# ai4co/rl4co

Measured on AMD Instinct MI355X. Metric: decode_steps_per_sec, higher is better.
Workload: dtype bf16; 1 GPU; BASELINE configs[1]: TSPEnv num_loc=100 batch=4096/GPU AttentionModel(3L,d128,h8) greedy rollout, bf16 encoder GEMMs, bf16 cache; leg=c2_greedy, batch_per_gpu=4096, cache_dtype=bf16, launch=pipeline, input=one synthetic batch resident in HBM, reused by every step, parallelism=replicas x1 (instances sharded)

## Files before the change

rl4co_amd/csrc/am_decode.hip:

```cpp
#include <hip/hip_runtime.h>

#include "common.h"
#include "rl4co_math.h"
#include "topkp.h"

namespace {

constexpr int kD = RL4CO_EMBED_DIM;
constexpr int kH = RL4CO_NUM_HEADS;
constexpr int kDH = kD / kH;
constexpr int kUnroll = 4;
constexpr float kNegInf = -__builtin_huge_valf();
constexpr float kSqrtD = 11.3137084989847604f;

struct CacheF32 {
  using elem = float;
  using raw = float4;
  static constexpr int EPL = 4;
  __device__ static inline raw zero() { return make_float4(0.f, 0.f, 0.f, 0.f); }
  __device__ static inline raw ld(const elem* p) { return *reinterpret_cast<const float4*>(p); }
  __device__ static inline void cvt(const raw& t, float (&v)[4]) {
    v[0] = t.x; v[1] = t.y; v[2] = t.z; v[3] = t.w;
  }
};
// ... 8 lines not shown
    v[0] = __uint_as_float(t.x << 16); v[1] = __uint_as_float(t.x & 0xffff0000u);
    v[2] = __uint_as_float(t.y << 16); v[3] = __uint_as_float(t.y & 0xffff0000u);
    v[4] = __uint_as_float(t.z << 16); v[5] = __uint_as_float(t.z & 0xffff0000u);
    v[6] = __uint_as_float(t.w << 16); v[7] = __uint_as_float(t.w & 0xffff0000u);
  }
};

struct CacheF16 {
  using elem = uint16_t;
  using raw = uint4;
  static constexpr int EPL = 8;
  typedef _Float16 half2_t __attribute__((ext_vector_type(2)));
  __device__ static inline raw zero() { return make_uint4(0u, 0u, 0u, 0u); }
  __device__ static inline raw ld(const elem* p) { return *reinterpret_cast<const uint4*>(p); }
  __device__ static inline void cvt(const raw& t, float (&v)[8]) {
    const half2_t a = __builtin_bit_cast(half2_t, t.x), b = __builtin_bit_cast(half2_t, t.y);
    const half2_t c = __builtin_bit_cast(half2_t, t.z), d = __builtin_bit_cast(half2_t, t.w);
    v[0] = (float)a[0]; v[1] = (float)a[1]; v[2] = (float)b[0]; v[3] = (float)b[1];
    v[4] = (float)c[0]; v[5] = (float)c[1]; v[6] = (float)d[0]; v[7] = (float)d[1];
  }
};

__host__ __device__ inline int lds_pad(int N) { return (N + 63) & ~63; }

template <class C>
struct CtxTables {
  const char *cur, *first;
  int64_t rs;
  bool half;
  __device__ inline CtxTables(const rl4co_am_decode_args& a, int cb, int N, int e0) {
    half = a.ctx_dtype != RL4CO_DT_F32;
    const int64_t esz = half ? 2 : 4;
    rs = (a.ctx_row_stride ? a.ctx_row_stride : (int64_t)kD) * esz;
    const int64_t off = ((int64_t)cb * (a.ctx_batch_stride ? a.ctx_batch_stride : (int64_t)N * kD) + e0) * esz;
    cur = a.ctx_cur ? static_cast<const char*>(a.ctx_cur) + off : nullptr;
    first = a.ctx_first ? static_cast<const char*>(a.ctx_first) + off : nullptr;
  }
  __device__ inline void load(const char* table, int64_t row, float (&v)[C::EPL]) const {
    const char* p = table + row * rs;
    if constexpr (sizeof(typename C::elem) == 2) {
      if (half) {
        C::cvt(C::ld(reinterpret_cast<const typename C::elem*>(p)), v);
        return;
      }
    }
#pragma unroll
    for (int e = 0; e < C::EPL; ++e) v[e] = reinterpret_cast<const float*>(p)[e];
  }
};

__device__ inline int trajectory_of_block(int b, int B, int B_inst) {
  const int S = B / B_inst;
  if (S == 1 || (B_inst & 7) != 0) return b;
  const int xcd = b & 7, k = b >> 3;
  return (k % S) * B_inst + (k / S) * 8 + xcd;
}

__device__ inline void wave_lds_sync() {
  __builtin_amdgcn_fence(__ATOMIC_RELEASE, "workgroup");
  __builtin_amdgcn_wave_barrier();
  __builtin_amdgcn_fence(__ATOMIC_ACQUIRE, "workgroup");
}

struct TrajState {
  int cur, first;
  long long step_i;
  float used;
  float time;
  bool done;
  uint32_t errbits;
  float ent_acc;
};

__device__ inline int build_list(const rl4co_am_decode_args& a, const uint8_t* mk, uint16_t* fl, int N, int lane) {
  int F = 0;
  if (a.mask_inner && a.mask_logits) {
    for (int j0 = 0; j0 < N; j0 += 64) {
      const int j = j0 + lane;
      const bool f = j < N && mk[j] != 0;
      const unsigned long long bal = __ballot(f);
      if (f) fl[F + __popcll(bal & ((1ull << lane) - 1ull))] = (uint16_t)j;
      F += __popcll(bal);
    }
  } else {
    for (int j = lane; j < N; j += 64) fl[j] = (uint16_t)j;
    F = N;
  }
  wave_lds_sync();
  return F;
}

template <int ENV>
__device__ inline int commit_and_step(const rl4co_am_decode_args& a, TrajState& st, float* lg, const uint16_t* fl, int F,
                                      uint8_t* mk, uint8_t* vis, const float* dem, float cap, int r, int t, int N, int lane,
                                      const float* oplocs, const float* opmax, const float* twdur, int bc);

template <int ENV, bool FILT = false>
__device__ inline int finalize_and_step(const rl4co_am_decode_args& a, TrajState& st, float* lg, float* xs,
                                        const uint16_t* fl, int F, uint8_t* mk, uint8_t* vis, const float* dem, float cap,
                                        int r, int t, int N, int lane, const float* oplocs = nullptr,
                                        const float* opmax = nullptr, const float* twdur = nullptr) {
  bool nan_seen = false;
  float zmax = kNegInf;
  for (int c = lane; c < F; c += 64) {
    float z = lg[c] / kSqrtD;
    if (z != z) nan_seen = true;
    if (a.tanh_clipping > 0.0f) z = rl4co_tanhf(z) * a.tanh_clipping;
    if (a.mask_logits && mk[fl[c]] == 0) z = kNegInf;
    if (a.temperature != 1.0f) z = z / a.temperature;
    lg[c] = z;
    zmax = fmaxf(zmax, z);
  }
  if (__any(nan_seen)) st.errbits |= RL4CO_EBIT_NAN_LOGIT;
  zmax = rl4co::bfly_max<1, 64>(zmax);
  float zsum = 0.0f;
  const int64_t tcol = (int64_t)a.t0 + t;
  constexpr bool filt = FILT;
  if (filt) {
    for (int c = lane; c < F; c += 64) xs[c] = rl4co_expf(lg[c] - zmax);
    zsum = rl4co::topkp_filter(lg, xs, F, a.top_k, a.top_p, lane);
    if (a.kept_bits)
      rl4co::topkp_write_bits(a.kept_bits + ((int64_t)r * a.out_stride + tcol) * a.kept_words, a.kept_words, lg, fl, F,
                              N, reinterpret_cast<uint32_t*>(xs + N), lane);
  } else {
    for (int c = lane; c < F; c += 64) zsum = zsum + rl4co_expf(lg[c] - zmax);
    zsum = rl4co::bfly_sum<1, 64>(zsum);
  }
  const float lse = rl4co_logf(zsum);

  float best = kNegInf;
  int bc = 0x7fffffff;
  float ent = 0.0f;
  float* alp = a.all_logps ? a.all_logps + ((int64_t)r * a.out_stride + tcol) * N : nullptr;
  if (alp && F < N) {
    for (int j = lane; j < N; j += 64)
      if (mk[j] == 0) alp[j] = kNegInf;
  }
  for (int c = lane; c < F; c += 64) {
    const int j = fl[c];
    const float lp = (lg[c] - zmax) - lse;
    lg[c] = lp;
    float key = lp;
    if (a.mode == RL4CO_DECODE_SAMPLE) {
      const float nz = a.exp_noise
                           ? a.exp_noise[((int64_t)t * a.B + r) * N + j]
                           : rl4co_exp1_noise(a.philox_seed ^ (a.philox_seed_dev ? *a.philox_seed_dev : 0ull),
                                              a.philox_offset + (uint64_t)tcol, (uint32_t)r,
                                              (uint32_t)j);
      key = rl4co_expf(lp) / nz;
      if (filt && !(lp > kNegInf)) key = kNegInf;
    }
    if (bc == 0x7fffffff || key > best) {
      best = key;
      bc = c;
    }
    if (a.entropy && lp > kNegInf) ent = fmaf(rl4co_expf(lp), lp, ent);
    if (alp) alp[j] = lp;
  }
  rl4co::bfly_argmax(best, bc);
  if (a.entropy) st.ent_acc = st.ent_acc - rl4co::bfly_sum<1, 64>(ent);
  wave_lds_sync();
  return commit_and_step<ENV>(a, st, lg, fl, F, mk, vis, dem, cap, r, t, N, lane, oplocs, opmax, twdur, bc);
}

template <int ENV>
__device__ inline int commit_and_step(const rl4co_am_decode_args& a, TrajState& st, float* lg, const uint16_t* fl, int F,
                                      uint8_t* mk, uint8_t* vis, const float* dem, float cap, int r, int t, int N, int lane,
                                      const float* oplocs, const float* opmax, const float* twdur, int bc) {
  const int64_t tcol = (int64_t)a.t0 + t;
  int bi;
  float logp;
  if (a.mode == RL4CO_DECODE_EVALUATE) {
    bi = (int)a.forced_actions[(int64_t)r * a.out_stride + tcol];
    if (bi < 0 || bi >= N) {
      st.errbits |= RL4CO_EBIT_INFEASIBLE;
      bi = 0;
    }
    int pos = 0x7fffffff;
    for (int c = lane; c < F; c += 64)
      if (fl[c] == bi) pos = c;
    pos = -rl4co::bfly_i_max(-pos);
    logp = pos < F ? lg[pos] : kNegInf;
  } else {
    bi = (bc < F) ? (int)fl[bc] : 0;
    logp = (bc < F) ? lg[bc] : kNegInf;
  }
  if (mk[bi] == 0) st.errbits |= RL4CO_EBIT_INFEASIBLE;
  if (!(logp > -1000.0f)) st.errbits |= RL4CO_EBIT_NEG_INF_LOGP;
  if (lane == 0) {
    a.actions[(int64_t)r * a.out_stride + tcol] = bi;
    a.logps[(int64_t)r * a.out_stride + tcol] = logp;
  }
  wave_lds_sync();

  if (ENV == RL4CO_ENV_TSP) {
    if (st.step_i == 0) st.first = bi;
    st.cur = bi;
    if (lane == 0) mk[bi] = 0;
    st.step_i += 1;
    wave_lds_sync();
    bool any_left = false;
    for (int j = lane; j < N; j += 64) any_left |= mk[j] != 0;
    st.done = !__any(any_left);
  } else if (ENV == RL4CO_ENV_PDP) {
    const int n = N - 1;
    if (lane == 0) {
      vis[bi] &= (uint8_t)~1u;
      vis[(bi + n / 2) % (n + 1)] |= 2;
    }
    st.step_i += 1;
    st.cur = bi;
    wave_lds_sync();
    bool left = false;
    for (int j = lane; j < N; j += 64) {
      const uint8_t v = vis[j];
      mk[j] = (v == 3) ? 1 : 0;
      left |= (v & 1) != 0;
    }
    st.done = !__any(left);
  } else if (ENV == RL4CO_ENV_PCTSP) {
    st.used = st.used + dem[bi];
    if (lane == 0) vis[bi] = 1;
    st.done = (bi == 0) && (st.step_i > 0);
    st.step_i += 1;
    st.cur = bi;
    wave_lds_sync();
    const bool depot_visited = vis[0] != 0;
    bool unvisited = false;
    for (int j = lane; j < N; j += 64) {
      if (j >= 1) {
        mk[j] = (vis[j] != 0 || depot_visited) ? 0 : 1;
        unvisited |= vis[j] == 0;
      }
    }
    unvisited = __any(unvisited);
    if (lane == 0) mk[0] = ((st.used < 1.0f) && unvisited) ? 0 : 1;
  } else if (ENV == RL4CO_ENV_OP) {
    const float cx = oplocs[2 * st.cur], cy = oplocs[2 * st.cur + 1];
    const float bx = oplocs[2 * bi], by = oplocs[2 * bi + 1];
    {
      const float dx = bx - cx, dy = by - cy;
      st.used = st.used + sqrtf(fmaf(dy, dy, dx * dx));
    }
    if (lane == 0) vis[bi] = 1;
    st.done = (bi == 0) && (st.step_i > 0);
    st.step_i += 1;
    st.cur = bi;
    wave_lds_sync();
    const bool depot_visited = vis[0] != 0;
    for (int j = lane; j < N; j += 64) {
      const float dx = oplocs[2 * j] - bx, dy = oplocs[2 * j + 1] - by;
      const bool exceeds = st.used + sqrtf(fmaf(dy, dy, dx * dx)) > opmax[j];
      mk[j] = (j == 0 || !(vis[j] != 0 || depot_visited || exceeds)) ? 1 : 0;
    }
  } else {
    if (ENV == RL4CO_ENV_CVRPTW) {
      const float dx = oplocs[2 * bi] - oplocs[2 * st.cur], dy = oplocs[2 * bi + 1] - oplocs[2 * st.cur + 1];
      const float served = fmaxf(st.time + sqrtf(fmaf(dy, dy, dx * dx)), opmax[2 * bi]) + twdur[bi];
      st.time = (bi != 0 ? 1.0f : 0.0f) * served;
    }
    const int di = min(max(bi - 1, 0), N - 2);
    st.used = (st.used + dem[di]) * (bi != 0 ? 1.0f : 0.0f);
    st.cur = bi;
    if (lane == 0) vis[bi] = 1;
    wave_lds_sync();
    const float thr = cap + 1e-5f;
    bool any_feasible = false, all_visited = true;
    for (int j = lane; j < N; j += 64) {
      all_visited &= vis[j] != 0;
      if (j >= 1) {
        const bool masked = (vis[j] != 0) || (dem[j - 1] + st.used > thr);
        mk[j] = masked ? 0 : 1;
        any_feasible |= !masked;
      }
    }
    any_feasible = __any(any_feasible);
    st.done = __all(all_visited);
    if (lane == 0) mk[0] = ((st.cur == 0) && any_feasible) ? 0 : 1;
    if (ENV == RL4CO_ENV_CVRPTW) {
      wave_lds_sync();
      const float bx = oplocs[2 * bi], by = oplocs[2 * bi + 1];
      for (int j = lane; j < N; j += 64) {
        const float dx = oplocs[2 * j] - bx, dy = oplocs[2 * j + 1] - by;
        if (!(st.time + sqrtf(fmaf(dy, dy, dx * dx)) <= opmax[2 * j + 1])) mk[j] = 0;
      }
    }
  }
  wave_lds_sync();
  return bi;
}

template <int EPL>
__device__ inline void gemv_t(float (&out)[EPL], const float* __restrict__ wt, const float* in_lds, int width, int e0) {
#pragma unroll
  for (int e = 0; e < EPL; ++e) out[e] = 0.0f;
  for (int k = 0; k < width; ++k) {
    const float c = in_lds[k];
#pragma unroll
    for (int e = 0; e < EPL; ++e) out[e] = fmaf(wt[(int64_t)k * kD + e0 + e], c, out[e]);
  }
}

constexpr int kRowCacheNone = 0xFF;
__host__ __device__ inline int row_cache_bytes(int N, int S, int esz) {
  return S > 0 ? S * 3 * kD * esz + lds_pad(N) + S : 0;
}

template <class C, int ENV, bool UNFOLD = false, bool FILT = false>
__global__ void __launch_bounds__(64) am_decode_kernel(const rl4co_am_decode_args a, const int S) {
  constexpr int EPL = C::EPL;
  constexpr int LPR = kD / EPL;
  constexpr int RPL = 64 / LPR;
  constexpr int LPH = kDH / EPL;
  constexpr bool kRowCache = !UNFOLD && (ENV == RL4CO_ENV_TSP || ENV == RL4CO_ENV_CVRP);
  using elem = typename C::elem;
  using raw_t = typename C::raw;

  extern __shared__ __align__(16) unsigned char smem[];
  const int lane = threadIdx.x;
  const int r = trajectory_of_block(blockIdx.x, a.B, a.B_inst);
  const int N = a.N;
  const int Np = lds_pad(N);
  float* sc = reinterpret_cast<float*>(smem);
  float* lg = sc + Np * kH;
  float* mh = lg + Np;
  uint16_t* fl = reinterpret_cast<uint16_t*>(mh + kH);
  uint8_t* mk = reinterpret_cast<uint8_t*>(fl + Np);
  uint8_t* vis = mk + Np;
  elem* rc = reinterpret_cast<elem*>(vis + Np);
  uint8_t* rslot = reinterpret_cast<uint8_t*>(rc + S * 3 * kD);
  uint8_t* rpend = rslot + Np;

  const int cb = r % a.B_inst;
  const int rg = lane / LPR;
  const int li = lane % LPR;
  const int hd = li / LPH;
  const int e0 = li * EPL;

  const elem* Kg = static_cast<const elem*>(a.glimpse_key) + (int64_t)cb * a.kvl_batch_stride + e0;
  const elem* Vg = static_cast<const elem*>(a.glimpse_val) + (int64_t)cb * a.kvl_batch_stride + e0;
  const elem* Kl = static_cast<const elem*>(a.logit_key) + (int64_t)cb * a.kvl_batch_stride + e0;
  const int64_t rs = a.kvl_row_stride;
  const CtxTables<C> ctx(a, cb, N, e0);
  const float* hrow = UNFOLD ? a.node_embed + (int64_t)cb * N * kD + e0 : nullptr;

  uint8_t* gmask = a.action_mask + (int64_t)r * N;
  for (int j = lane; j < Np; j += 64) mk[j] = (j < N) ? gmask[j] : (uint8_t)0;
  constexpr bool kScalarCtx = ENV == RL4CO_ENV_CVRP || ENV == RL4CO_ENV_OP || ENV == RL4CO_ENV_PCTSP || ENV == RL4CO_ENV_CVRPTW;
  constexpr bool kCvrpLike = ENV == RL4CO_ENV_CVRP || ENV == RL4CO_ENV_CVRPTW;
  if (ENV == RL4CO_ENV_PDP) {
    const uint8_t* gv = a.visited + (int64_t)r * N;
    const uint8_t* gt = a.to_deliver + (int64_t)r * N;
    for (int j = lane; j < Np; j += 64) vis[j] = (j < N) ? (uint8_t)((gv[j] != 0 ? 1 : 0) | (gt[j] != 0 ? 2 : 0)) : (uint8_t)0;
  } else if (ENV != RL4CO_ENV_TSP) {
    const uint8_t* gv = a.visited + (int64_t)r * N;
    for (int j = lane; j < Np; j += 64) vis[j] = (j < N) ? gv[j] : (uint8_t)1;
  }
  TrajState st;
  st.cur = (int)a.current_node[r];
  st.first = (ENV == RL4CO_ENV_TSP) ? (int)a.first_node[r] : 0;
  st.step_i = !kCvrpLike ? a.step_i[r] : 0;
  st.time = (ENV == RL4CO_ENV_CVRPTW) ? a.current_time[r] : 0.0f;
  st.used = kScalarCtx ? a.used_capacity[r] : 0.0f;
  st.done = a.done[r] != 0;
  st.errbits = 0;
  st.ent_acc = 0.0f;
  const float* oplocs = (ENV == RL4CO_ENV_OP || ENV == RL4CO_ENV_CVRPTW) ? a.locs + (int64_t)cb * N * 2 : nullptr;
  const float* opmax = (ENV == RL4CO_ENV_OP)       ? a.max_length + (int64_t)cb * N
                       : (ENV == RL4CO_ENV_CVRPTW) ? a.time_windows + (int64_t)cb * N * 2
                                                   : nullptr;
  const float* twdur = (ENV == RL4CO_ENV_CVRPTW) ? a.durations + (int64_t)cb * N : nullptr;
  const float cap = (kCvrpLike || ENV == RL4CO_ENV_PCTSP) ? a.vehicle_capacity[r]
                                                                      : ((ENV == RL4CO_ENV_OP) ? opmax[0] : 0.0f);
  const float* dem = kCvrpLike                  ? a.demand + (int64_t)cb * (N - 1)
                     : (ENV == RL4CO_ENV_PCTSP) ? a.demand + (int64_t)cb * N
                                                : nullptr;
  wave_lds_sync();

  const bool list_all = !(a.mask_inner && a.mask_logits);
  auto candidate = [&](int j) -> bool {
    return list_all || (ENV == RL4CO_ENV_TSP ? mk[j] != 0 : (j == 0 || vis[j] == 0));
  };
  const bool caching = kRowCache && S > 0;
  if (caching) {
    for (int j = lane; j < Np; j += 64) rslot[j] = (uint8_t)kRowCacheNone;
    wave_lds_sync();
    int k = 0;
    for (int j0 = N - 1; j0 >= 0 && k < S; j0 -= 64) {
      const int j = j0 - lane;
      const bool f = j >= 0 && candidate(j);
      const unsigned long long bal = __ballot(f);
      const int s = k + __popcll(bal & ((1ull << lane) - 1ull));
      if (f && s < S) {
        rslot[j] = (uint8_t)s;
        rpend[s] = 1;
      }
      k += __popcll(bal);
    }
    wave_lds_sync();
  }
  auto lds_row = [&](int j, int plane) -> const elem* { return rc + (rslot[j] * 3 + plane) * kD + e0; };
  auto fill_row = [&](int j, int plane, const raw_t& v) {
    const int s = rslot[j];
    if (s != kRowCacheNone) *reinterpret_cast<raw_t*>(rc + (s * 3 + plane) * kD + e0) = v;
  };

  float qb[EPL];
#pragma unroll
  for (int e = 0; e < EPL; ++e) qb[e] = a.q_bias ? a.q_bias[(int64_t)cb * kD + e0 + e] : 0.0f;

  const bool single = a.max_steps == 1;
  int t = 0;
  int rows_read = 0;

  for (; t < a.max_steps && (!st.done || single); ++t) {
    const int F = build_list(a, mk, fl, N, lane);
    int hend = F, pbeg = F;
    if (caching) {
      const int c_lo = max(F - S, 0);
      int last_hbm = c_lo - 1, first_pend = F;
      for (int c = c_lo + lane; c < F; c += 64) {
        const int s = rslot[fl[c]];
        const bool pend = s != kRowCacheNone && rpend[s] != 0;
        if (s == kRowCacheNone || pend) last_hbm = c;
        if (pend) first_pend = min(first_pend, c);
      }
      hend = rl4co::bfly_i_max(last_hbm) + 1;
      pbeg = -rl4co::bfly_i_max(-first_pend);
    }
    rows_read += hend;

    float q[EPL];
    if constexpr (UNFOLD) {
      float* cv = sc;
      if (rg == 0) {
        if (ENV == RL4CO_ENV_TSP) {
          const bool ph = st.step_i < 1;
#pragma unroll
          for (int e = 0; e < EPL; ++e) {
            cv[e0 + e] = ph ? a.w_placeholder[e0 + e] : hrow[(int64_t)st.first * kD + e];
            cv[kD + e0 + e] = ph ? a.w_placeholder[kD + e0 + e] : hrow[(int64_t)st.cur * kD + e];
          }
        } else {
#pragma unroll
          for (int e = 0; e < EPL; ++e) cv[e0 + e] = hrow[(int64_t)st.cur * kD + e];
          if (li == 0) cv[kD] = cap - st.used;
        }
      }
      wave_lds_sync();
      gemv_t<EPL>(q, a.w_ctx_t, cv, a.ctx_width, e0);
#pragma unroll
      for (int e = 0; e < EPL; ++e) q[e] = q[e] + qb[e];
      wave_lds_sync();
    } else if (ENV == RL4CO_ENV_TSP) {
      if (st.step_i < 1) {
#pragma unroll
        for (int e = 0; e < EPL; ++e) q[e] = a.q_step0[e0 + e] + qb[e];
      } else {
        float cf[EPL], cc[EPL];
        ctx.load(ctx.first, st.first, cf);
        ctx.load(ctx.cur, st.cur, cc);
#pragma unroll
        for (int e = 0; e < EPL; ++e) q[e] = (cf[e] + cc[e]) + qb[e];
      }
    } else if (ENV == RL4CO_ENV_PDP) {
      float cc[EPL];
      ctx.load(ctx.cur, st.cur, cc);
#pragma unroll
      for (int e = 0; e < EPL; ++e) q[e] = cc[e] + qb[e];
    } else {
      float rem = cap - st.used;
      if (ENV == RL4CO_ENV_PCTSP && !(rem > 0.0f)) rem = 0.0f;
      float cc[EPL];
      ctx.load(ctx.cur, st.cur, cc);
#pragma unroll
      for (int e = 0; e < EPL; ++e) {
        float v = fmaf(a.w_cap[e0 + e], rem, cc[e]);
        if (ENV == RL4CO_ENV_CVRPTW) v = fmaf(a.w_time[e0 + e], st.time, v);
        q[e] = v + qb[e];
      }
    }
#pragma unroll
    for (int e = 0; e < EPL; ++e) q[e] = q[e] * 0.25f;

    float m = kNegInf;
    auto score = [&](const raw_t& rw, int c, int j) {
      const bool valid = j >= 0;
      float k[EPL];
      C::cvt(rw, k);
      float acc = 0.0f;
#pragma unroll
      for (int e = 0; e < EPL; ++e) acc = fmaf(q[e], k[e], acc);
      acc = rl4co::bfly_sum<1, LPH>(acc);
      const bool feas = valid && (!a.mask_inner || mk[valid ? j : 0] != 0);
      const float sv = feas ? acc : kNegInf;
      if (valid && (li % LPH) == 0) sc[c * kH + hd] = sv;
      m = fmaxf(m, sv);
    };
    for (int c0 = 0; c0 < F; c0 += RPL * kUnroll) {
      raw_t rw[kUnroll];
      int jj[kUnroll];
#pragma unroll
      for (int u = 0; u < kUnroll; ++u) {
        const int c = c0 + u * RPL + rg;
        jj[u] = (c < F) ? (int)fl[c] : -1;
        rw[u] = (jj[u] < 0) ? C::zero() : (c < hend ? C::ld(Kg + (int64_t)jj[u] * rs) : C::ld(lds_row(jj[u], 0)));
      }
#pragma unroll
      for (int u = 0; u < kUnroll; ++u) {
        const int c = c0 + u * RPL + rg;
        if (caching && c >= pbeg && c < hend) fill_row(jj[u], 0, rw[u]);
        score(rw[u], c, jj[u]);
      }
    }
    m = rl4co::bfly_max<LPR, 64>(m);
    if (rg == 0 && (li % LPH) == 0) mh[hd] = m;
    wave_lds_sync();
    {
      const float mm = mh[lane & (kH - 1)];
      for (int idx = lane; idx < F * kH; idx += 64) sc[idx] = rl4co_expf(sc[idx] - mm);
    }
    wave_lds_sync();

    float l = 0.0f;
    float o[EPL];
#pragma unroll
    for (int e = 0; e < EPL; ++e) o[e] = 0.0f;
    auto accumulate = [&](const raw_t& rw, int c, bool ok) {
      float v[EPL];
      C::cvt(rw, v);
      const float p = ok ? sc[c * kH + hd] : 0.0f;
      l = l + p;
#pragma unroll
      for (int e = 0; e < EPL; ++e) o[e] = fmaf(p, v[e], o[e]);
    };
    for (int c0 = 0; c0 < F; c0 += RPL * kUnroll) {
      raw_t rw[kUnroll];
      bool ok[kUnroll];
#pragma unroll
      for (int u = 0; u < kUnroll; ++u) {
        const int c = c0 + u * RPL + rg;
        ok[u] = c < F;
        rw[u] = !ok[u] ? C::zero() : (c < hend ? C::ld(Vg + (int64_t)fl[c] * rs) : C::ld(lds_row(fl[c], 1)));
      }
#pragma unroll
      for (int u = 0; u < kUnroll; ++u) {
        const int c = c0 + u * RPL + rg;
        if (caching && c >= pbeg && c < hend) fill_row(fl[c], 1, rw[u]);
        accumulate(rw[u], c, ok[u]);
      }
    }
    l = 1.0f / rl4co::bfly_sum<LPR, 64>(l);
#pragma unroll
    for (int e = 0; e < EPL; ++e) o[e] = rl4co::bfly_sum<LPR, 64>(o[e]) * l;
    if constexpr (UNFOLD) {
      wave_lds_sync();
      if (rg == 0) {
#pragma unroll
        for (int e = 0; e < EPL; ++e) sc[e0 + e] = o[e];
      }
      wave_lds_sync();
      gemv_t<EPL>(o, a.w_out_t, sc, kD, e0);
    }

    auto logit = [&](const raw_t& rw, int c) {
      float k[EPL];
      C::cvt(rw, k);
      float acc = 0.0f;
#pragma unroll
      for (int e = 0; e < EPL; ++e) acc = fmaf(o[e], k[e], acc);
      acc = rl4co::bfly_sum<1, LPR>(acc);
      if (c < F && li == 0) lg[c] = acc;
    };
    for (int c0 = 0; c0 < F; c0 += RPL * kUnroll) {
      raw_t rw[kUnroll];
#pragma unroll
      for (int u = 0; u < kUnroll; ++u) {
        const int c = c0 + u * RPL + rg;
        rw[u] = (c >= F) ? C::zero() : (c < hend ? C::ld(Kl + (int64_t)fl[c] * rs) : C::ld(lds_row(fl[c], 2)));
      }
#pragma unroll
      for (int u = 0; u < kUnroll; ++u) {
        const int c = c0 + u * RPL + rg;
        if (caching && c >= pbeg && c < hend) fill_row(fl[c], 2, rw[u]);
        logit(rw[u], c);
      }
    }
    if (caching) {
      for (int c = pbeg + lane; c < hend; c += 64) {
        const int s = rslot[fl[c]];
        if (s != kRowCacheNone) rpend[s] = 0;
      }
    }
    wave_lds_sync();

    const int bi = finalize_and_step<ENV, FILT>(a, st, lg, sc, fl, F, mk, vis, dem, cap, r, t, N, lane, oplocs, opmax, twdur);
    if (caching && rslot[bi] != kRowCacheNone && !candidate(bi)) {
      int nxt = -1;
      for (int j = lane; j < N; j += 64)
        if (candidate(j) && rslot[j] == kRowCacheNone) nxt = j;
      nxt = rl4co::bfly_i_max(nxt);
      const int s = rslot[bi];
      wave_lds_sync();
      if (lane == 0) {
        rslot[bi] = (uint8_t)kRowCacheNone;
        if (nxt >= 0) {
          rslot[nxt] = (uint8_t)s;
          rpend[s] = 1;
        }
      }
      wave_lds_sync();
    }
  }
  if (!single && !st.done && t >= a.max_steps) st.errbits |= RL4CO_EBIT_MAX_STEPS;

  for (int j = lane; j < N; j += 64) gmask[j] = mk[j];
  if (ENV == RL4CO_ENV_PDP) {
    uint8_t* gv = a.visited + (int64_t)r * N;
    uint8_t* gt = a.to_deliver + (int64_t)r * N;
    for (int j = lane; j < N; j += 64) {
      gv[j] = vis[j] & 1;
      gt[j] = (vis[j] >> 1) & 1;
    }
  } else if (ENV != RL4CO_ENV_TSP) {
    uint8_t* gv = a.visited + (int64_t)r * N;
    for (int j = lane; j < N; j += 64) gv[j] = vis[j];
  }
  if (lane == 0) {
    a.current_node[r] = st.cur;
    a.done[r] = st.done ? 1 : 0;
    if (ENV == RL4CO_ENV_TSP) a.first_node[r] = st.first;
    if (!kCvrpLike) a.step_i[r] = st.step_i;
    if (ENV == RL4CO_ENV_CVRPTW) a.current_time[r] = st.time;
    if (kScalarCtx) a.used_capacity[r] = st.used;
    if (a.n_steps) a.n_steps[r] = t;
    if (a.steps_summary) {
      atomicMax(a.steps_summary, t);
      atomicAdd(a.steps_summary + 1, t);
      atomicAdd(reinterpret_cast<unsigned long long*>(a.steps_summary + 2), (unsigned long long)rows_read);
    }
    if (a.entropy) a.entropy[r] += st.ent_acc;
    if (st.errbits) atomicOr(a.err, (int)st.errbits);
  }
}

constexpr int kLdsWaves = 4;
constexpr int kLdsGroups = 16;

template <int ENV, bool FILT = false>
__device__ inline int wide_scores(const rl4co_am_decode_args& a, TrajState& st, float* lg, const uint16_t* fl, int F,
                                  const uint8_t* mk, float* xs, int nw, int r, int t, int N, int tid) {
  constexpr int T = 64 * kLdsWaves;
  const int w = tid >> 6, lane = tid & 63;
  float* ex = xs;
  float* xw = xs + 2 * nw;
  bool nan_seen = false;
  float zmax = kNegInf;
  for (int c = tid; c < F; c += T) {
    float z = lg[c] / kSqrtD;
    if (z != z) nan_seen = true;
    if (a.tanh_clipping > 0.0f) z = rl4co_tanhf(z) * a.tanh_clipping;
    if (a.mask_logits && mk[fl[c]] == 0) z = kNegInf;
    if (a.temperature != 1.0f) z = z / a.temperature;
    lg[c] = z;
    zmax = fmaxf(zmax, z);
  }
  zmax = rl4co::bfly_max<1, 64>(zmax);
  const bool wave_nan = __any(nan_seen);
  if (lane == 0) {
    xw[w] = zmax;
    xw[4 + w] = wave_nan ? 1.0f : 0.0f;
  }
  __syncthreads();
  zmax = fmaxf(fmaxf(xw[0], xw[1]), fmaxf(xw[2], xw[3]));
  if ((xw[4] + xw[5]) + (xw[6] + xw[7]) != 0.0f) st.errbits |= RL4CO_EBIT_NAN_LOGIT;
  for (int c = tid; c < F; c += T) ex[c] = rl4co_expf(lg[c] - zmax);
  __syncthreads();
  const int64_t tcol = (int64_t)a.t0 + t;
  constexpr bool filt = FILT;
  if (w == 0) {
    float zsum = 0.0f;
    if (filt) {
      zsum = rl4co::topkp_filter(lg, ex, F, a.top_k, a.top_p, lane);
      if (a.kept_bits)
        rl4co::topkp_write_bits(a.kept_bits + ((int64_t)r * a.out_stride + tcol) * a.kept_words, a.kept_words, lg, fl,
                                F, N, reinterpret_cast<uint32_t*>(xw + 16), lane);
    } else {
      for (int c = lane; c < F; c += 64) zsum = zsum + ex[c];
      zsum = rl4co::bfly_sum<1, 64>(zsum);
    }
    if (lane == 0) xw[8] = rl4co_logf(zsum);
  }
  __syncthreads();
  const float lse = xw[8];
  float* alp = a.all_logps ? a.all_logps + ((int64_t)r * a.out_stride + tcol) * N : nullptr;
  if (alp && F < N) {
    for (int j = tid; j < N; j += T)
      if (mk[j] == 0) alp[j] = kNegInf;
  }
  for (int c = tid; c < F; c += T) {
    const int j = fl[c];
    const float lp = (lg[c] - zmax) - lse;
    lg[c] = lp;
    float key = lp;
    if (a.mode == RL4CO_DECODE_SAMPLE) {
      const float nz = a.exp_noise
                           ? a.exp_noise[((int64_t)t * a.B + r) * N + j]
                           : rl4co_exp1_noise(a.philox_seed ^ (a.philox_seed_dev ? *a.philox_seed_dev : 0ull),
                                              a.philox_offset + (uint64_t)tcol, (uint32_t)r,
                                              (uint32_t)j);
      key = rl4co_expf(lp) / nz;
      if (filt && !(lp > kNegInf)) key = kNegInf;
    }
    ex[c] = key;
    if (alp) alp[j] = lp;
  }
  __syncthreads();
  int bc = 0x7fffffff;
  if (w == 0) {
    float best = kNegInf, ent = 0.0f;
    for (int c = lane; c < F; c += 64) {
      const float key = ex[c];
      if (bc == 0x7fffffff || key > best) {
        best = key;
        bc = c;
      }
      if (a.entropy) {
        const float lp = lg[c];
        if (lp > kNegInf) ent = fmaf(rl4co_expf(lp), lp, ent);
      }
    }
    rl4co::bfly_argmax(best, bc);
    if (a.entropy) st.ent_acc = st.ent_acc - rl4co::bfly_sum<1, 64>(ent);
    wave_lds_sync();
  }
  return bc;
}

__host__ __device__ inline int lds_variant_sc_rows(int N) { return N < 80 ? 80 : N; }
__host__ __device__ inline int wide_scratch_bytes(int N) {
  const int nw = (N + 3) & ~3;
  return lds_variant_sc_rows(N) * kH * 4 + nw * 4 + kLdsWaves * kH * 4 + 32 + 2 * nw + 2 * nw;
}
__host__ __device__ inline int lds_variant_bytes(int N) { return 3 * N * kD * 2 + wide_scratch_bytes(N); }

template <int ENV, bool RESIDENT, class C = CacheBF16, bool FILT = false>
__global__ void __launch_bounds__(64 * kLdsWaves, 4) am_decode_wide_kernel(const rl4co_am_decode_args a) {
  constexpr int EPL = 8, LPR = 16, LPH = 2;
  constexpr int U = 4;
  extern __shared__ __align__(16) unsigned char smem[];
  const int tid = threadIdx.x;
  const int w = tid >> 6, lane = tid & 63;
  const int r = trajectory_of_block(blockIdx.x, a.B, a.B_inst);
  const int N = a.N;
  const int nw = (N + 3) & ~3;
  uint16_t* planes = reinterpret_cast<uint16_t*>(smem);
  float* sc = reinterpret_cast<float*>(planes + (RESIDENT ? 3 * N * kD : 0));
  float* lg = sc + lds_variant_sc_rows(N) * kH;
  float* mpart = lg + nw;
  int* shi = reinterpret_cast<int*>(mpart + kLdsWaves * kH);
  uint16_t* fl = reinterpret_cast<uint16_t*>(shi + 8);
  uint8_t* mk = reinterpret_cast<uint8_t*>(fl + nw);
  uint8_t* vis = mk + nw;

  const int cb = r % a.B_inst;
  const int rg = lane / LPR, li = lane % LPR, hd = li / LPH, e0 = li * EPL;
  const uint16_t *Kg, *Vg, *Kl;
  int64_t rs;
  if constexpr (RESIDENT) {
    Kg = planes + e0;
    Vg = planes + N * kD + e0;
    Kl = planes + 2 * N * kD + e0;
    rs = kD;
  } else {
    Kg = static_cast<const uint16_t*>(a.glimpse_key) + (int64_t)cb * a.kvl_batch_stride + e0;
    Vg = static_cast<const uint16_t*>(a.glimpse_val) + (int64_t)cb * a.kvl_batch_stride + e0;
    Kl = static_cast<const uint16_t*>(a.logit_key) + (int64_t)cb * a.kvl_batch_stride + e0;
    rs = a.kvl_row_stride;
  }
  const CtxTables<C> ctx(a, cb, N, e0);
  auto opart = [&](int wv, int d) -> float* { return sc + ((16 * (d >> 5) + 4 * wv) * kH) + (d & 31); };
  auto lpart = [&](int wv, int h) -> float* { return sc + ((16 * 4 + 4 * wv) * kH) + h; };

  if constexpr (RESIDENT) {
    const uint16_t* src[3] = {static_cast<const uint16_t*>(a.glimpse_key), static_cast<const uint16_t*>(a.glimpse_val),
                              static_cast<const uint16_t*>(a.logit_key)};
    const int chunks = N * (kD / 8);
    for (int p = 0; p < 3; ++p) {
      const uint16_t* g = src[p] + (int64_t)cb * a.kvl_batch_stride;
      for (int c = tid; c < chunks; c += 64 * kLdsWaves) {
        const int row = c >> 4, col = (c & 15) * 8;
        *reinterpret_cast<uint4*>(planes + (p * N + row) * kD + col) =
            *reinterpret_cast<const uint4*>(g + (int64_t)row * a.kvl_row_stride + col);
      }
    }
  }
  constexpr bool kScalarCtx = ENV == RL4CO_ENV_CVRP || ENV == RL4CO_ENV_OP || ENV == RL4CO_ENV_PCTSP || ENV == RL4CO_ENV_CVRPTW;
  constexpr bool kCvrpLike = ENV == RL4CO_ENV_CVRP || ENV == RL4CO_ENV_CVRPTW;
  uint8_t* gmask = a.action_mask + (int64_t)r * N;
  for (int j = tid; j < nw; j += 64 * kLdsWaves) mk[j] = (j < N) ? gmask[j] : (uint8_t)0;
  if (ENV == RL4CO_ENV_PDP) {
    const uint8_t* gv = a.visited + (int64_t)r * N;
    const uint8_t* gt = a.to_deliver + (int64_t)r * N;
    for (int j = tid; j < nw; j += 64 * kLdsWaves)
      vis[j] = (j < N) ? (uint8_t)((gv[j] != 0 ? 1 : 0) | (gt[j] != 0 ? 2 : 0)) : (uint8_t)0;
  } else if (ENV != RL4CO_ENV_TSP) {
    const uint8_t* gv = a.visited + (int64_t)r * N;
    for (int j = tid; j < nw; j += 64 * kLdsWaves) vis[j] = (j < N) ? gv[j] : (uint8_t)1;
  }
  TrajState st;
  st.cur = (int)a.current_node[r];
  st.first = (ENV == RL4CO_ENV_TSP) ? (int)a.first_node[r] : 0;
  st.step_i = !kCvrpLike ? a.step_i[r] : 0;
  st.time = (ENV == RL4CO_ENV_CVRPTW) ? a.current_time[r] : 0.0f;
  st.used = kScalarCtx ? a.used_capacity[r] : 0.0f;
  st.done = a.done[r] != 0;
  st.errbits = 0;
  st.ent_acc = 0.0f;
  const float* oplocs = (ENV == RL4CO_ENV_OP || ENV == RL4CO_ENV_CVRPTW) ? a.locs + (int64_t)cb * N * 2 : nullptr;
  const float* opmax = (ENV == RL4CO_ENV_OP)       ? a.max_length + (int64_t)cb * N
                       : (ENV == RL4CO_ENV_CVRPTW) ? a.time_windows + (int64_t)cb * N * 2
                                                   : nullptr;
  const float* twdur = (ENV == RL4CO_ENV_CVRPTW) ? a.durations + (int64_t)cb * N : nullptr;
  const float cap = (kCvrpLike || ENV == RL4CO_ENV_PCTSP) ? a.vehicle_capacity[r] : ((ENV == RL4CO_ENV_OP) ? opmax[0] : 0.0f);
  const float* dem = kCvrpLike                  ? a.demand + (int64_t)cb * (N - 1)
                     : (ENV == RL4CO_ENV_PCTSP) ? a.demand + (int64_t)cb * N
                                                : nullptr;
  __syncthreads();
  if (w == 0) {
    const int F0 = build_list(a, mk, fl, N, lane);
    if (lane == 0) shi[2] = F0;
  }
  __syncthreads();

  float qb[EPL];
#pragma unroll
  for (int e = 0; e < EPL; ++e) qb[e] = a.q_bias ? a.q_bias[(int64_t)cb * kD + e0 + e] : 0.0f;

  const bool single = a.max_steps == 1;
  int t = 0;
  int rows_read = 0;

  for (; t < a.max_steps && (!st.done || single); ++t) {
    const int F = shi[2];
    rows_read += F;
    const int iters = (F + kLdsGroups - 1) / kLdsGroups;
    float q[EPL];
    if (ENV == RL4CO_ENV_TSP) {
      if (st.step_i < 1) {
#pragma unroll
        for (int e = 0; e < EPL; ++e) q[e] = a.q_step0[e0 + e] + qb[e];
      } else {
        float cf[EPL], cc[EPL];
        ctx.load(ctx.first, st.first, cf);
        ctx.load(ctx.cur, st.cur, cc);
#pragma unroll
        for (int e = 0; e < EPL; ++e) q[e] = (cf[e] + cc[e]) + qb[e];
      }
    } else if (ENV == RL4CO_ENV_PDP) {
      float cc[EPL];
      ctx.load(ctx.cur, st.cur, cc);
#pragma unroll
      for (int e = 0; e < EPL; ++e) q[e] = cc[e] + qb[e];
    } else {
      float rem = cap - st.used;
      if (ENV == RL4CO_ENV_PCTSP && !(rem > 0.0f)) rem = 0.0f;
      float cc[EPL];
      ctx.load(ctx.cur, st.cur, cc);
#pragma unroll
      for (int e = 0; e < EPL; ++e) {
        float v = fmaf(a.w_cap[e0 + e], rem, cc[e]);
        if (ENV == RL4CO_ENV_CVRPTW) v = fmaf(a.w_time[e0 + e], st.time, v);
        q[e] = v + qb[e];
      }
    }
#pragma unroll
    for (int e = 0; e < EPL; ++e) q[e] = q[e] * 0.25f;

    float m = kNegInf;
    for (int i0 = 0; i0 < iters; i0 += U) {
      uint4 rw[U];
      int jj[U];
#pragma unroll
      for (int u = 0; u < U; ++u) {
        const int c = kLdsGroups * (i0 + u) + 4 * w + rg;
        jj[u] = (c < F) ? (int)fl[c] : -1;
        rw[u] = (jj[u] >= 0) ? *reinterpret_cast<const uint4*>(Kg + (int64_t)jj[u] * rs) : C::zero();
      }
#pragma unroll
      for (int u = 0; u < U; ++u) {
// ... 349 lines not shown
```

Measured before the change: 140.2 million instance·step/s.

## Precompute packed per-candidate entry table and add fast gather path in decode

Builds a per-step packed uint32 entry table in LDS that encodes node index, cache slot, LDS/fill/missing/infeasible flags. The three K/V/L walks then share one templated walker instead of each re-reading the list, slot and mask arrays. A fast path uses 24-bit multiply offsets with no branches for the prefix of rows that come from HBM. The kernel also sets waves_per_eu(4), reads the kernarg pointer each step to cut SGPR pressure, and uses readfirstlane on the bounds. This reduces per-row address and branch overhead and register pressure, at the cost of an extra LDS pass and aliasing the logit buffer as the entry table.

```diff
diff --git a/rl4co_amd/csrc/am_decode.hip b/rl4co_amd/csrc/am_decode.hip
--- a/rl4co_amd/csrc/am_decode.hip
+++ b/rl4co_amd/csrc/am_decode.hip
@@ -334,12 +334,20 @@
 }
 
 constexpr int kRowCacheNone = 0xFF;
+
+constexpr uint32_t kEntNode = 0xFFFFu;
+constexpr int kEntSlotShift = 16;
+constexpr uint32_t kEntMissing = 1u << 24;
+constexpr uint32_t kEntLds = 1u << 25;
+constexpr uint32_t kEntFill = 1u << 26;
+constexpr uint32_t kEntInfeas = 1u << 27;
 __host__ __device__ inline int row_cache_bytes(int N, int S, int esz) {
   return S > 0 ? S * 3 * kD * esz + lds_pad(N) + S : 0;
 }
 
 template <class C, int ENV, bool UNFOLD = false, bool FILT = false>
-__global__ void __launch_bounds__(64) am_decode_kernel(const rl4co_am_decode_args a, const int S) {
+__global__ void __launch_bounds__(64) __attribute__((amdgpu_waves_per_eu(4))) am_decode_kernel(const rl4co_am_decode_args a_launch, const int S) {
+  const rl4co_am_decode_args& a = a_launch;
   constexpr int EPL = C::EPL;
   constexpr int LPR = kD / EPL;
   constexpr int RPL = 64 / LPR;
@@ -369,10 +377,13 @@
   const int hd = li / LPH;
   const int e0 = li * EPL;
 
-  const elem* Kg = static_cast<const elem*>(a.glimpse_key) + (int64_t)cb * a.kvl_batch_stride + e0;
-  const elem* Vg = static_cast<const elem*>(a.glimpse_val) + (int64_t)cb * a.kvl_batch_stride + e0;
-  const elem* Kl = static_cast<const elem*>(a.logit_key) + (int64_t)cb * a.kvl_batch_stride + e0;
+  const elem* Kg = static_cast<const elem*>(a.glimpse_key) + (int64_t)cb * a.kvl_batch_stride;
+  const elem* Vg = static_cast<const elem*>(a.glimpse_val) + (int64_t)cb * a.kvl_batch_stride;
+  const elem* Kl = static_cast<const elem*>(a.logit_key) + (int64_t)cb * a.kvl_batch_stride;
   const int64_t rs = a.kvl_row_stride;
+  const bool narrow = rs * (int64_t)sizeof(elem) < (1 << 24) && (int64_t)N * rs * (int64_t)sizeof(elem) < (1ll << 32);
+  const uint32_t rsb = (uint32_t)(rs * (int64_t)sizeof(elem));
+  const uint32_t e0b = (uint32_t)(e0 * (int)sizeof(elem));
   const CtxTables<C> ctx(a, cb, N, e0);
   const float* hrow = UNFOLD ? a.node_embed + (int64_t)cb * N * kD + e0 : nullptr;
 
@@ -431,21 +442,22 @@
     }
     wave_lds_sync();
   }
-  auto lds_row = [&](int j, int plane) -> const elem* { return rc + (rslot[j] * 3 + plane) * kD + e0; };
-  auto fill_row = [&](int j, int plane, const raw_t& v) {
-    const int s = rslot[j];
-    if (s != kRowCacheNone) *reinterpret_cast<raw_t*>(rc + (s * 3 + plane) * kD + e0) = v;
-  };
-
   float qb[EPL];
 #pragma unroll
   for (int e = 0; e < EPL; ++e) qb[e] = a.q_bias ? a.q_bias[(int64_t)cb * kD + e0 + e] : 0.0f;
 
+  constexpr int kBatch = RPL * kUnroll;
+  uint32_t* ent = reinterpret_cast<uint32_t*>(lg);
+  const bool need_feas = a.mask_inner && !a.mask_logits;
   const bool single = a.max_steps == 1;
   int t = 0;
   int rows_read = 0;
 
-  for (; t < a.max_steps && (!st.done || single); ++t) {
+  const int max_steps = a.max_steps;
+  for (; t < max_steps && (!st.done || single); ++t) {
+    auto ka = __builtin_amdgcn_kernarg_segment_ptr();
+    asm volatile("" : "+s"(ka));
+    const rl4co_am_decode_args& a = *(const rl4co_am_decode_args*)ka;
     const int F = build_list(a, mk, fl, N, lane);
     int hend = F, pbeg = F;
     if (caching) {
@@ -457,10 +469,61 @@
         if (s == kRowCacheNone || pend) last_hbm = c;
         if (pend) first_pend = min(first_pend, c);
       }
-      hend = rl4co::bfly_i_max(last_hbm) + 1;
-      pbeg = -rl4co::bfly_i_max(-first_pend);
+      hend = __builtin_amdgcn_readfirstlane(rl4co::bfly_i_max(last_hbm)) + 1;
+      pbeg = -__builtin_amdgcn_readfirstlane(rl4co::bfly_i_max(-first_pend));
     }
     rows_read += hend;
+    for (int c = lane; c < (F + kBatch - 1) / kBatch * kBatch; c += 64) {
+      uint32_t w = kEntMissing;
+      if (c < F) {
+        const int j = fl[c];
+        w = (uint32_t)j;
+        if (caching && c >= F - S) {
+          const uint32_t s = rslot[j];
+          if (s != (uint32_t)kRowCacheNone && c >= hend) w |= (s << kEntSlotShift) | kEntLds;
+          else if (s != (uint32_t)kRowCacheNone && c >= pbeg) w |= (s << kEntSlotShift) | kEntFill;
+        }
+        if (need_feas && mk[j] == 0) w |= kEntInfeas;
+      }
+      ent[c] = w;
+    }
+    wave_lds_sync();
+    const int fast_end = (!UNFOLD && narrow && !need_feas) ? min(pbeg, hend) : 0;
+    auto walk = [&](const int plane, const elem* base, auto&& fn) {
+      int c0 = 0;
+      for (; c0 + kBatch <= fast_end; c0 += kBatch) {
+        uint32_t w[kUnroll];
+        raw_t rw[kUnroll];
+#pragma unroll
+        for (int u = 0; u < kUnroll; ++u) w[u] = ent[c0 + u * RPL + rg];
+#pragma unroll
+        for (int u = 0; u < kUnroll; ++u)
+          rw[u] = C::ld(reinterpret_cast<const elem*>(reinterpret_cast<const char*>(base) + (__umul24(w[u], rsb) + e0b)));
+#pragma unroll
+        for (int u = 0; u < kUnroll; ++u) fn(rw[u], c0 + u * RPL + rg, true, true);
+      }
+      for (; c0 < F; c0 += kBatch) {
+        uint32_t w[kUnroll];
+        raw_t rw[kUnroll];
+#pragma unroll
+        for (int u = 0; u < kUnroll; ++u) w[u] = ent[c0 + u * RPL + rg];
+#pragma unroll
+        for (int u = 0; u < kUnroll; ++u) {
+          rw[u] = C::zero();
+          if ((w[u] & (kEntMissing | kEntLds)) == 0) {
+            rw[u] = C::ld(base + ((int64_t)(w[u] & kEntNode) * rs + e0));
+          } else if (kRowCache && (w[u] & kEntLds) != 0) {
+            rw[u] = C::ld(rc + (((w[u] >> kEntSlotShift) & 0xFFu) * 3 + plane) * kD + e0);
+          }
+        }
+#pragma unroll
+        for (int u = 0; u < kUnroll; ++u) {
+          if (kRowCache && (w[u] & kEntFill) != 0)
+            *reinterpret_cast<raw_t*>(rc + (((w[u] >> kEntSlotShift) & 0xFFu) * 3 + plane) * kD + e0) = rw[u];
+          fn(rw[u], c0 + u * RPL + rg, (w[u] & kEntMissing) == 0, (w[u] & (kEntMissing | kEntInfeas)) == 0);
+        }
+      }
+    };
 
     float q[EPL];
     if constexpr (UNFOLD) {
@@ -516,35 +579,17 @@
     for (int e = 0; e < EPL; ++e) q[e] = q[e] * 0.25f;
 
     float m = kNegInf;
-    auto score = [&](const raw_t& rw, int c, int j) {
-      const bool valid = j >= 0;
+    walk(0, Kg, [&](const raw_t& rw, int c, bool valid, bool feas) {
       float k[EPL];
       C::cvt(rw, k);
       float acc = 0.0f;
 #pragma unroll
       for (int e = 0; e < EPL; ++e) acc = fmaf(q[e], k[e], acc);
       acc = rl4co::bfly_sum<1, LPH>(acc);
-      const bool feas = valid && (!a.mask_inner || mk[valid ? j : 0] != 0);
       const float sv = feas ? acc : kNegInf;
       if (valid && (li % LPH) == 0) sc[c * kH + hd] = sv;
       m = fmaxf(m, sv);
-    };
-    for (int c0 = 0; c0 < F; c0 += RPL * kUnroll) {
-      raw_t rw[kUnroll];
-      int jj[kUnroll];
-#pragma unroll
-      for (int u = 0; u < kUnroll; ++u) {
-        const int c = c0 + u * RPL + rg;
-        jj[u] = (c < F) ? (int)fl[c] : -1;
-        rw[u] = (jj[u] < 0) ? C::zero() : (c < hend ? C::ld(Kg + (int64_t)jj[u] * rs) : C::ld(lds_row(jj[u], 0)));
-      }
-#pragma unroll
-      for (int u = 0; u < kUnroll; ++u) {
-        const int c = c0 + u * RPL + rg;
-        if (caching && c >= pbeg && c < hend) fill_row(jj[u], 0, rw[u]);
-        score(rw[u], c, jj[u]);
-      }
-    }
+    });
     m = rl4co::bfly_max<LPR, 64>(m);
     if (rg == 0 && (li % LPH) == 0) mh[hd] = m;
     wave_lds_sync();
@@ -558,30 +603,14 @@
     float o[EPL];
 #pragma unroll
     for (int e = 0; e < EPL; ++e) o[e] = 0.0f;
-    auto accumulate = [&](const raw_t& rw, int c, bool ok) {
+    walk(1, Vg, [&](const raw_t& rw, int c, bool valid, bool) {
       float v[EPL];
       C::cvt(rw, v);
-      const float p = ok ? sc[c * kH + hd] : 0.0f;
+      const float p = valid ? sc[c * kH + hd] : 0.0f;
       l = l + p;
 #pragma unroll
       for (int e = 0; e < EPL; ++e) o[e] = fmaf(p, v[e], o[e]);
-    };
-    for (int c0 = 0; c0 < F; c0 += RPL * kUnroll) {
-      raw_t rw[kUnroll];
-      bool ok[kUnroll];
-#pragma unroll
-      for (int u = 0; u < kUnroll; ++u) {
-        const int c = c0 + u * RPL + rg;
-        ok[u] = c < F;
-        rw[u] = !ok[u] ? C::zero() : (c < hend ? C::ld(Vg + (int64_t)fl[c] * rs) : C::ld(lds_row(fl[c], 1)));
-      }
-#pragma unroll
-      for (int u = 0; u < kUnroll; ++u) {
-        const int c = c0 + u * RPL + rg;
-        if (caching && c >= pbeg && c < hend) fill_row(fl[c], 1, rw[u]);
-        accumulate(rw[u], c, ok[u]);
-      }
-    }
+    });
     l = 1.0f / rl4co::bfly_sum<LPR, 64>(l);
 #pragma unroll
     for (int e = 0; e < EPL; ++e) o[e] = rl4co::bfly_sum<LPR, 64>(o[e]) * l;
@@ -595,29 +624,15 @@
       gemv_t<EPL>(o, a.w_out_t, sc, kD, e0);
     }
 
-    auto logit = [&](const raw_t& rw, int c) {
+    walk(2, Kl, [&](const raw_t& rw, int c, bool valid, bool) {
       float k[EPL];
       C::cvt(rw, k);
       float acc = 0.0f;
 #pragma unroll
       for (int e = 0; e < EPL; ++e) acc = fmaf(o[e], k[e], acc);
       acc = rl4co::bfly_sum<1, LPR>(acc);
-      if (c < F && li == 0) lg[c] = acc;
-    };
-    for (int c0 = 0; c0 < F; c0 += RPL * kUnroll) {
-      raw_t rw[kUnroll];
-#pragma unroll
-      for (int u = 0; u < kUnroll; ++u) {
-        const int c = c0 + u * RPL + rg;
-        rw[u] = (c >= F) ? C::zero() : (c < hend ? C::ld(Kl + (int64_t)fl[c] * rs) : C::ld(lds_row(fl[c], 2)));
-      }
-#pragma unroll
-      for (int u = 0; u < kUnroll; ++u) {
-        const int c = c0 + u * RPL + rg;
-        if (caching && c >= pbeg && c < hend) fill_row(fl[c], 2, rw[u]);
-        logit(rw[u], c);
-      }
-    }
+      if (valid && li == 0) ent[c] = __float_as_uint(acc);
+    });
     if (caching) {
       for (int c = pbeg + lane; c < hend; c += 64) {
         const int s = rslot[fl[c]];
```

Measured after the change: 138.0 million instance·step/s. 1.6% lower.
